# UW-ACL/SCPToolbox.jl

Measured on NVIDIA H100. Metric: SCP iterations/sec (batch), higher is better.
Workload: dtype f64

## Files before the change

scptoolbox.jl_b200/csrc/conic_ipm.cuh:

```cuda
#pragma once
#include <cuda_runtime.h>
#include <math_constants.h>

#include "conic_sn.cuh"

struct IpmProgram {
    int n, p, m, l, nsoc, nk, nnzL, nlevels, nwm, nnzA, nnzG;
    const int *soc_dim, *soc_off, *soc_woff;
    const int *A_rp, *A_ci, *G_rp, *G_ci;
    const int *At_rp, *At_ri, *At_vi, *Gt_rp, *Gt_ri, *Gt_vi;
    const int *iperm;
    const int *L_cp, *L_ri, *Lr_rp, *Lr_pos, *Lr_col;
    const int *lvl_ptr, *lvl_nodes;
    const int *as_ptr, *as_a, *as_b, *as_c, *as_src, *as_sign;
    const int4 *fw_item, *bw_item;
    const int4 *fwp_item, *bwp_item, *fa_item, *fb_item;
    SnProgram sn;
    HyProgram hy;
    int ysize;
    const int *sn_pos;
    const int *fa_lvl, *fa_R, *fb_lvl;
    const int *fwp_lvl, *bwp_lvl, *fwp_R, *bwp_R;
    const int2 *Lr_pc, *ft_op;
    const int4 *fwc_item, *bwc_item;
// ... 28 lines not shown
    double *xw, *yw, *zw, *sw;
    int *warm;
    double *rx, *ry, *rz, *lam, *wm, *socw, *soceta;
    double *dx, *dy, *dz, *ds, *dsa, *dza, *tm, *gm, *r1, *r2, *e1, *e2, *rhs, *Y, *Ls, *Lrow, *invD;
    double *part;
    double *pcnt;
    int vsmem;
    int psmem;
    double *pobj, *dobj, *res;
    int *status, *iters;
    const int *skip;
    int debug_kkt;
    int lvl_prof;
    int sn;
    long long *prof;
    double *trace;
    int trace_seed;
};

enum { IPM_OPTIMAL = 0, IPM_MAXIT = 1, IPM_NUMERICAL = 2, IPM_ALMOST = 3, IPM_PINF = 4, IPM_DINF = 5 };

#define IPM_MAXG 8
#define IPM_NT_MAX 1024

#ifdef CONIC_IPM_IMPL
struct Ctx {
    int G, sg, slot, nslots, tid, nwarps;
    int R, rr, isl, nisl;
    const int *s_lvl;
    int o_fal, o_faR, o_fbl;
    int o_fwl, o_bwl, o_fwR, o_bwR, o_vs;
    int Rmax;
    int *flag;
    long long t_fw, t_bw, t_ldl_n;
    long long *lprof;
    int sn;
    double *Ypanels;
    const struct SnArgs *s_sn;
    const struct HyArgs *s_hy;
    size_t ysize;
    const int *s_done;
    double *s_delta;
    int *s_bad;
    double rho_min, bad_abs;
    double *vs;
    double *Lrow;
    double *fpart, *spart;
    unsigned *pcnt;
    double reftol;
    const double *s_mu;
    double mu_tight;
    double *red;
    double *out;
};

template <int K>
__device__ __forceinline__ void seed_reduce(const Ctx &c, double (&v)[K], int op)
{
    const int lane = c.tid & 31, warp = c.tid >> 5;
    const int G = c.G;
#pragma unroll
    for (int k = 0; k < K; k++) {
        double a = v[k];
        for (int o = 16; o >= G; o >>= 1) {
            const double t = __shfl_xor_sync(0xffffffffu, a, o);
            a = (op == 0) ? a + t : ((op == 1) ? fmin(a, t) : fmax(a, t));
        }
        v[k] = a;
    }
    __syncthreads();
    if (lane < G) {
#pragma unroll
        for (int k = 0; k < K; k++) c.red[(k * (IPM_NT_MAX / 32) + warp) * IPM_MAXG + lane] = v[k];
    }
    __syncthreads();
    if (c.tid < G) {
#pragma unroll
        for (int k = 0; k < K; k++) {
            double a = c.red[(k * (IPM_NT_MAX / 32)) * IPM_MAXG + c.tid];
            for (int w = 1; w < c.nwarps; w++) {
                const double t = c.red[(k * (IPM_NT_MAX / 32) + w) * IPM_MAXG + c.tid];
                a = (op == 0) ? a + t : ((op == 1) ? fmin(a, t) : fmax(a, t));
            }
            c.out[k * IPM_MAXG + c.tid] = a;
        }
    }
    __syncthreads();
}

#define GI(e) ((size_t)(e) * G + sg)

__device__ __forceinline__ void set_lanes(Ctx &c, int R)
{
    const int sh = 31 - __clz(R);
    c.R = R; c.rr = c.slot & (R - 1); c.isl = c.slot >> sh; c.nisl = c.nslots >> sh;
}

__device__ __forceinline__ double lanes_sum(const Ctx &c, double a)
{
    for (int o = c.G; o < c.G * c.R; o <<= 1) a += __shfl_xor_sync(0xffffffffu, a, o);
    return a;
}

__device__ __forceinline__ double row_dot(const int *rp, const int *ci, const double *Mv, const double *x, int r,
                                          int G, int sg)
{
    double acc = 0.0;
    for (int k = rp[r]; k < rp[r + 1]; k++) acc = fma(Mv[GI(k)], x[GI(ci[k])], acc);
    return acc;
}
__device__ __forceinline__ double col_dot(const int *trp, const int *tri, const int *tvi, const double *Mv,
                                          const double *y, int v, int G, int sg)
{
    double acc = 0.0;
    for (int k = trp[v]; k < trp[v + 1]; k++) acc = fma(Mv[GI(tvi[k])], y[GI(tri[k])], acc);
    return acc;
}

__device__ void apply_winv2(const IpmProgram &P, const Ctx &c, const double *wm, const double *socw,
                            const double *soceta, const double *in, double *out)
{
    const int G = c.G, sg = c.sg;
    for (int r = c.slot; r < P.l; r += c.nslots) out[GI(r)] = wm[GI(r)] * in[GI(r)];
    for (int k = c.slot; k < P.nsoc; k += c.nslots) {
// ... 30 lines not shown
    for (int t = c.slot; t < ntgt; t += c.nslots) {
        double acc = dl * (double)P.as_sign[t];
        const int src = P.as_src[t];
        if (src >= 0) acc += Av[GI(src)];
        for (int k = P.as_ptr[t]; k < P.as_ptr[t + 1]; k++)
            acc = fma(Gv[GI(P.as_a[k])] * Gv[GI(P.as_b[k])], wmx[GI(P.as_c[k])], acc);
        if (D.sn) Y[(size_t)sg * c.ysize + P.sn_pos[t]] = acc;
        else Y[GI(t)] = acc;
    }
    __syncthreads();
}

#define IPM_FPF CONIC_FACTOR_PF
__device__ __forceinline__ bool ipm_split_done(double *part, unsigned *cnt, int4 e, double v, int G, int sg)
{
    part[e.w * G + sg] = v;
    __threadfence_block();
    const bool last = atomicAdd(&cnt[e.y * G + sg], 1u) == (unsigned)(e.z - e.y - 1);
    if (last) { __threadfence_block(); cnt[e.y * G + sg] = 0u; }
    return last;
}
__device__ __forceinline__ double ipm_split_sum(const double *part, int k0, int k1, double acc, int G, int sg)
{
    for (int k = k0; k < k1; k++) acc -= part[k * G + sg];
    return acc;
}
struct FactorArgs {
    const int4 *fa_item, *fb_item;
    const int2 *ft_op;
    const int4 *fb_cmb;
    double *Y, *Ls, *Lrow, *invD;
    double *part;
    int o_fal, o_faR, o_fbl;
    int nl, nnzLd, G, sg, slot, nslots;
    long long *lprof;
};
extern __shared__ int ipm_smem[];
__shared__ double ipm_s_delta[IPM_MAXG];
__shared__ int ipm_s_bad[IPM_MAXG];
__shared__ double ipm_s_reg[2];

__device__ __noinline__ void kkt_factor_levels(const FactorArgs a)
{
    __builtin_assume(__isGlobal(a.fa_item)); __builtin_assume(__isGlobal(a.fb_item)); __builtin_assume(__isGlobal(a.ft_op));
    __builtin_assume(__isGlobal(a.Y)); __builtin_assume(__isGlobal(a.Ls)); __builtin_assume(__isGlobal(a.Lrow));
    __builtin_assume(__isGlobal(a.invD));
    const int *fal = ipm_smem + a.o_fal, *faR = ipm_smem + a.o_faR, *fbl = ipm_smem + a.o_fbl;
    const int G = a.G, sg = a.sg, slot = a.slot, nslots = a.nslots;
    int t_tgt;
    int2 t_op[IPM_FPF];
    int i_tgt, i_k0, i_k1;
#define IPM_FA_ITEM(LV, OFF)                                                              \
    {                                                                                     \
        const int R_ = faR[LV], sh_ = 31 - __clz(R_);                                     \
        const int w_ = fal[LV] + (OFF) + (slot >> sh_);                                   \
        i_tgt = -1; i_k0 = 0; i_k1 = 0;                                                   \
        if ((OFF) < fal[(LV) + 1] - fal[LV] && w_ < fal[(LV) + 1]) {                      \
            const int4 it_ = a.fa_item[w_];                                               \
            i_tgt = it_.w ? ((it_.w - 1) | (1 << 30)) : it_.x;                              \
            i_k0 = it_.y + (slot & (R_ - 1)); i_k1 = it_.z;                               \
        }                                                                                 \
    }
#define IPM_FA_OPS(TGT, OP, R_)                                                           \
    {                                                                                     \
        TGT = i_tgt;                                                                      \
        _Pragma("unroll") for (int j = 0; j < IPM_FPF; j++) {                             \
            const int k_ = i_k0 + j * (R_);                                               \
            OP[j] = (i_tgt >= 0 && k_ < i_k1) ? a.ft_op[k_] : make_int2(-1, 0);           \
        }                                                                                 \
    }
    IPM_FA_ITEM(0, 0)
    IPM_FA_OPS(t_tgt, t_op, faR[0])
    IPM_FA_ITEM(0, (nslots >> (31 - __clz(faR[0]))))
    long long tl_ = a.lprof ? clock64() : 0;
    for (int lv = 0; lv < a.nl; lv++) {
        const int R = faR[lv], nisl = nslots >> (31 - __clz(R));
        const int nA = fal[lv + 1] - fal[lv];
        const int b0 = fbl[lv], b1 = fbl[lv + 1];
        int4 sc = make_int4(-1, 0, 0, 0), sr = make_int4(0, 0, 0, 0);
        if (b0 + slot < b1) { sc = a.fb_item[b0 + slot]; sr = a.fb_cmb[b0 + slot]; }
        for (int off = 0; off < nA; off += nisl) {
            double ya_[IPM_FPF], la_[IPM_FPF];
#pragma unroll
            for (int j = 0; j < IPM_FPF; j++) {
                const bool on_ = t_op[j].x >= 0;
                ya_[j] = on_ ? __ldcg(&a.Y[(size_t)t_op[j].x * G + sg]) : 0.0;
                la_[j] = on_ ? a.Lrow[(size_t)t_op[j].y * G + sg] : 0.0;
            }
            int n_tgt; int2 n_op[IPM_FPF];
            IPM_FA_OPS(n_tgt, n_op, R)
            IPM_FA_ITEM(lv, off + 2 * nisl)
            double part_ = 0.0;
#pragma unroll
            for (int j = 0; j < IPM_FPF; j++) part_ = fma(ya_[j], la_[j], part_);
            for (int o_ = G; o_ < G * R; o_ <<= 1) part_ += __shfl_xor_sync(0xffffffffu, part_, o_);
            if (t_tgt >= 0 && (slot & (R - 1)) == 0) {
                if (t_tgt >> 30) a.part[(t_tgt & 0x3fffffff) * G + sg] = part_;
                else { double *p_ = &a.Y[(size_t)t_tgt * G + sg]; *p_ = __ldcg(p_) - part_; }
            }
            t_tgt = n_tgt;
#pragma unroll
            for (int j = 0; j < IPM_FPF; j++) t_op[j] = n_op[j];
        }
        if (lv + 1 < a.nl) IPM_FA_ITEM(lv + 1, 0)
        __syncthreads();
        for (int w = b0 + slot; w < b1; w += nslots) {
            const double sgn = (sc.w & 1) ? 1.0 : -1.0;
            const bool isd = (sc.w & 2) != 0;
            double e = __ldcg(&a.Y[(size_t)sc.x * G + sg]);
            double d = isd ? 0.0 : __ldcg(&a.Y[(size_t)(a.nnzLd + sc.y) * G + sg]);
            const int4 cur = sc, cr = sr;
            if (w + nslots < b1) { sc = a.fb_item[w + nslots]; sr = a.fb_cmb[w + nslots]; }
            e = ipm_split_sum(a.part, cr.x, cr.y, e, G, sg);
            if (isd) d = e;
            else {
                d = ipm_split_sum(a.part, cr.z, cr.w, d, G, sg);
                if (cr.y > cr.x) a.Y[(size_t)cur.x * G + sg] = e;
                if (cur.w & 4) continue;
            }
            const double dl_ = ipm_s_delta[sg];
            if (!(sgn * d > 0.5 * dl_)) {
                if (isd && !(fabs(d) <= ipm_s_reg[1])) ipm_s_bad[sg] = 1;
                d = sgn * fmax(dl_, ipm_s_reg[0]);
            }
            const double inv = 1.0 / d;
            if (isd) a.invD[(size_t)cur.y * G + sg] = inv;
            else {
                const double lv_ = e * inv;
                a.Ls[(size_t)cur.x * G + sg] = lv_;
                a.Lrow[(size_t)cur.z * G + sg] = lv_;
            }
        }
        if (lv + 1 < a.nl) {
            const int Rn = faR[lv + 1];
            IPM_FA_OPS(t_tgt, t_op, Rn)
            IPM_FA_ITEM(lv + 1, (nslots >> (31 - __clz(Rn))))
        }
        __syncthreads();
        if (a.lprof) { const long long tn = clock64(); a.lprof[lv] += tn - tl_; tl_ = tn; }
    }
#undef IPM_FA_ITEM
#undef IPM_FA_OPS
}

struct SnArgs {
    SnProgram sn;
    double *Y, *invD, *vs;
    const int *s_done;
    const double *s_delta;
    int *s_bad;
    double rho_min, bad_abs;
    size_t ysize;
    int G, tid, nwarps, nls;
    long long *lprof;
};

template <int GS, class F>
__device__ __forceinline__ void sn_for_items(const SnArgs &a, int lv, int cls, F &&f)
{
    const int i0 = a.sn.cls_ptr[5 * lv + cls], nit = (a.sn.cls_ptr[5 * lv + cls + 1] - i0) * a.G;
    const int gsh = 31 - __clz(a.G);
    int unit, nunits;
    if (GS == 1) { unit = a.tid; nunits = a.nwarps * 32; }
    else { constexpr int GPW = 32 / (GS == 1 ? 32 : GS); unit = (a.tid >> 5) * GPW + ((a.tid & 31) / (GS == 1 ? 32 : GS)); nunits = a.nwarps * GPW; }
    int it = unit;
    int4 d0 = make_int4(0, 0, 0, 0), d1 = d0;
    if (it < nit) { const int q = 2 * (i0 + (it >> gsh)); d0 = a.sn.desc[q]; d1 = a.sn.desc[q + 1]; }
    while (it < nit) {
        const int sgi = it & (a.G - 1);
        const int4 c0 = d0, c1 = d1;
        const int nx = it + nunits;
        if (nx < nit) { const int q = 2 * (i0 + (nx >> gsh)); d0 = a.sn.desc[q]; d1 = a.sn.desc[q + 1]; }
        if (!a.s_done[sgi]) f(c0, c1, sgi);
        it = nx;
    }
// ... 25 lines not shown
}

template <int DIR>
__device__ __noinline__ void kkt_sweep_sn(const SnArgs *ap, int tid)
{
    SnArgs a = *ap;
    a.tid = tid;
    if (tid != 0) a.lprof = nullptr;
    const int G = a.G;
    double *vs = a.vs;
    long long tlp_ = a.lprof ? clock64() : 0;
    for (int st = 0; st < a.sn.nlevels; st++) {
        const int lv = DIR > 0 ? st : a.sn.nlevels - 1 - st;
        if (DIR > 0) {
            sn_for_items<1>(a, lv, 0, [&](const int4 d0, const int4 d1, int sgi) { sn1_forward_panel(a.sn, d0, d1, a.Y + (size_t)sgi * a.ysize, vs, G, sgi); });
            sn_for_items<8>(a, lv, 1, [&](const int4 d0, const int4 d1, int sgi) { sn_forward_panel<8>(a.sn, d0, d1, a.Y + (size_t)sgi * a.ysize, vs, G, sgi); });
            sn_for_items<16>(a, lv, 2, [&](const int4 d0, const int4 d1, int sgi) { sn_forward_panel<16>(a.sn, d0, d1, a.Y + (size_t)sgi * a.ysize, vs, G, sgi); });
            sn_for_items<32>(a, lv, 3, [&](const int4 d0, const int4 d1, int sgi) { sn_forward_panel<32>(a.sn, d0, d1, a.Y + (size_t)sgi * a.ysize, vs, G, sgi); });
        } else {
            sn_for_items<1>(a, lv, 0, [&](const int4 d0, const int4 d1, int sgi) { sn1_backward_panel(a.sn, d0, d1, a.Y + (size_t)sgi * a.ysize, vs, G, sgi); });
            sn_for_items<8>(a, lv, 1, [&](const int4 d0, const int4 d1, int sgi) { sn_backward_panel<8>(a.sn, d0, d1, a.Y + (size_t)sgi * a.ysize, vs, G, sgi); });
            sn_for_items<16>(a, lv, 2, [&](const int4 d0, const int4 d1, int sgi) { sn_backward_panel<16>(a.sn, d0, d1, a.Y + (size_t)sgi * a.ysize, vs, G, sgi); });
            sn_for_items<32>(a, lv, 3, [&](const int4 d0, const int4 d1, int sgi) { sn_backward_panel<32>(a.sn, d0, d1, a.Y + (size_t)sgi * a.ysize, vs, G, sgi); });
        }
        __syncthreads();
        if (a.lprof) { const long long tn = clock64(); a.lprof[(DIR > 0 ? 1 : 2) * a.nls + lv] += tn - tlp_; tlp_ = tn; }
    }
}

__device__ __forceinline__ void kkt_ldl_solve_sn(const IpmProgram &P, Ctx &c, const double *invD, double *v)
{
    const int G = c.G, sg = c.sg;
    double *vs = c.vs;
    const long long t0_ = clock64();
    for (int i = c.slot; i < P.nk; i += c.nslots) vs[i * G + sg] = v[GI(i)];
    __syncthreads();
    kkt_sweep_sn<1>(c.s_sn, c.tid);
    const long long t1_ = clock64();
    for (int i = c.slot; i < P.nk; i += c.nslots) vs[i * G + sg] *= invD[GI(i)];
    __syncthreads();
    kkt_sweep_sn<-1>(c.s_sn, c.tid);
    for (int i = c.slot; i < P.nk; i += c.nslots) v[GI(i)] = vs[i * G + sg];
    __syncthreads();
    const long long t2_ = clock64();
    c.t_fw += t1_ - t0_; c.t_bw += t2_ - t1_; c.t_ldl_n += 1;
}

struct HyArgs {
    HyProgram hy;
    double *Y, *Ls, *invD;
    const int *s_done;
    const double *s_delta;
    int *s_bad;
    double rho_min, bad_abs;
    int o_vs, nnzL, G, nwarps;
    long long *lprof;
};

template <class F>
__device__ __forceinline__ void hy_for_items(const HyArgs &a, int tl, int tid, F &&f)
{
    const int i0 = a.hy.tl_ptr[tl], nit = (a.hy.tl_ptr[tl + 1] - i0) * a.G;
    const int gsh = 31 - __clz(a.G);
    int it = tid >> 5;
    int4 d0 = make_int4(0, 0, 0, 0), d1 = d0;
    if (it < nit) { const int q = 2 * (i0 + (it >> gsh)); d0 = a.hy.desc[q]; d1 = a.hy.desc[q + 1]; }
    while (it < nit) {
        const int sgi = it & (a.G - 1);
        const int4 c0 = d0, c1 = d1;
        const int nx = it + a.nwarps;
        if (nx < nit) { const int q = 2 * (i0 + (nx >> gsh)); d0 = a.hy.desc[q]; d1 = a.hy.desc[q + 1]; }
        if (!a.s_done[sgi]) f(c0, c1, sgi);
        it = nx;
    }
}

__device__ __noinline__ void kkt_factor_top(const HyArgs *ap, int tid)
{
    const HyArgs a = *ap;
    long long *lp = (tid == 0) ? a.lprof : nullptr;
    long long tl_ = lp ? clock64() : 0;
    for (int tl = 0; tl < a.hy.ntl; tl++) {
        hy_for_items(a, tl, tid, [&](const int4 d0, const int4 d1, int sgi) {
            const double dl = a.s_delta[sgi];
            hy_factor_panel<32>(d0, d1, a.hy.upd_dst, a.Y, a.Ls, a.invD, a.nnzL, a.G, sgi, 0.5 * dl, fmax(dl, a.rho_min), a.bad_abs,
                                &a.s_bad[sgi]); });
        __syncthreads();
        if (lp) { const long long tn = clock64(); lp[tl] += tn - tl_; tl_ = tn; }
    }
}

template <int DIR>
__device__ __noinline__ void kkt_sweep_top(const HyArgs *ap, int tid)
{
    const HyArgs a = *ap;
    double *vs = (double *)(ipm_smem + a.o_vs);
    long long *lp = (tid == 0 && a.lprof) ? a.lprof + (DIR > 0 ? 1 : 2) * a.hy.ntl : nullptr;
    long long tl_ = lp ? clock64() : 0;
    for (int st = 0; st < a.hy.ntl; st++) {
        const int tl = DIR > 0 ? st : a.hy.ntl - 1 - st;
        if (DIR > 0) hy_for_items(a, tl, tid, [&](const int4 d0, const int4 d1, int sgi) { hy_forward_panel<32>(d0, d1, a.hy.rows, a.Ls, vs, a.G, sgi); });
        else hy_for_items(a, tl, tid, [&](const int4 d0, const int4 d1, int sgi) { hy_backward_panel<32>(d0, d1, a.hy.rows, a.Ls, vs, a.G, sgi); });
        __syncthreads();
        if (lp) { const long long tn = clock64(); lp[tl] += tn - tl_; tl_ = tn; }
    }
}

template <int SN>
__device__ __forceinline__ void kkt_factor(const IpmProgram &P, Ctx &c, double *Y, double *Ls, double *invD)
{
    if constexpr (SN == 1) { kkt_factor_sn(c.s_sn, c.tid); return; }
    FactorArgs a;
    a.fa_item = P.fa_item; a.fb_item = P.fb_item; a.ft_op = P.ft_op; a.fb_cmb = P.fb_cmb;
    a.Y = Y; a.Ls = Ls; a.Lrow = c.Lrow; a.invD = invD; a.part = c.fpart;
    a.o_fal = c.o_fal; a.o_faR = c.o_faR; a.o_fbl = c.o_fbl;
    a.nl = P.nlevels; a.nnzLd = P.nnzL; a.G = c.G; a.sg = c.sg; a.slot = c.slot; a.nslots = c.nslots;
    a.lprof = c.lprof;
    kkt_factor_levels(a);
    if constexpr (SN == 2) kkt_factor_top(c.s_hy, c.tid);
}

#define IPM_PF CONIC_SOLVE_PF
struct SweepArgs {
    const int4 *items;
    const int *idxarr;
    const double *vals;
    const int4 *cmb;
    double *part;
    unsigned *pcnt;
    int o_lvl, o_R, o_vs;
    int nl, lv0, G, sg, slot, nslots;
    long long *lprof;
};

template <int DIR>
__device__ __noinline__ void solve_sweep(const SweepArgs a)
{
    __builtin_assume(__isGlobal(a.items)); __builtin_assume(__isGlobal(a.idxarr)); __builtin_assume(__isGlobal(a.vals));
    const int *lvl = ipm_smem + a.o_lvl, *Rl = ipm_smem + a.o_R;
    double *vs = (double *)(ipm_smem + a.o_vs);
    const int G = a.G, sg = a.sg, slot = a.slot;
    const int nsteps = DIR > 0 ? a.nl - a.lv0 : a.lv0 + 1;
    if (nsteps <= 0) return;
    int i_node, i_k0, i_k1, i_R;
    int q_node;
    int q_idx[IPM_PF];
    double q_val[IPM_PF];
#define IPM_ITEM_LOAD(LV, OFF)                                                            \
    {                                                                                     \
        const int R_ = Rl[LV], sh_ = 31 - __clz(R_);                                      \
        const int w_ = lvl[LV] + (OFF) + (slot >> sh_);                                   \
        i_node = -1; i_R = R_; i_k0 = 0; i_k1 = 0;                                        \
        if (w_ < lvl[(LV) + 1]) {                                                         \
            const int4 it_ = a.items[w_];                                                 \
            i_node = it_.w ? ((it_.w - 1) | (1 << 30)) : it_.x;                             \
            i_k0 = it_.y + (slot & (R_ - 1)); i_k1 = it_.z;                               \
        }                                                                                 \
    }
#define IPM_VALS_LOAD()                                                                   \
    {                                                                                     \
        q_node = i_node;                                                                  \
        _Pragma("unroll") for (int j = 0; j < IPM_PF; j++) {                              \
            const int k_ = i_k0 + j * i_R;                                                \
            const bool on_ = i_node >= 0 && k_ < i_k1;                                    \
            q_idx[j] = on_ ? a.idxarr[k_] : 0;                                            \
            q_val[j] = on_ ? a.vals[(size_t)k_ * G + sg] : 0.0;                           \
        }                                                                                 \
    }
#define IPM_CONSUME(R)                                                                    \
    {                                                                                     \
        double part_ = 0.0;                                                               \
        _Pragma("unroll") for (int j = 0; j < IPM_PF; j++) part_ = fma(q_val[j], vs[q_idx[j] * G + sg], part_); \
        for (int o_ = G; o_ < G * (R); o_ <<= 1) part_ += __shfl_xor_sync(0xffffffffu, part_, o_); \
        if (q_node >= 0 && (slot & ((R) - 1)) == 0) {                                     \
            if (q_node >> 30) {                                                           \
                const int4 e_ = a.cmb[q_node & 0x3fffffff];                               \
                if (ipm_split_done(a.part, a.pcnt, e_, part_, G, sg))                     \
                    vs[e_.x * G + sg] = ipm_split_sum(a.part, e_.y, e_.z, vs[e_.x * G + sg], G, sg); \
            } else vs[q_node * G + sg] -= part_;                                          \
        }                                                                                 \
    }
    IPM_ITEM_LOAD(a.lv0, 0)
    IPM_VALS_LOAD()
    if (nsteps > 1) IPM_ITEM_LOAD(a.lv0 + DIR, 0) else i_node = -1;
    __syncthreads();
    long long tl_ = a.lprof ? clock64() : 0;
    for (int st = 0, lv = a.lv0; st < nsteps; st++, lv += DIR) {
        const int R = Rl[lv], nisl = a.nslots >> (31 - __clz(R));
        IPM_CONSUME(R)
        const int nit = lvl[lv + 1] - lvl[lv];
        if (nit > nisl) {
            const int sn = i_node, s0 = i_k0, s1 = i_k1, sR = i_R;
            for (int off = nisl; off < nit; off += nisl) {
                IPM_ITEM_LOAD(lv, off)
                IPM_VALS_LOAD()
                IPM_CONSUME(R)
            }
            i_node = sn; i_k0 = s0; i_k1 = s1; i_R = sR;
        }
        IPM_VALS_LOAD()
        if (st + 2 < nsteps) IPM_ITEM_LOAD(lv + 2 * DIR, 0) else i_node = -1;
        __syncthreads();
        if (a.lprof) { const long long tn = clock64(); a.lprof[lv] += tn - tl_; tl_ = tn; }
    }
#undef IPM_ITEM_LOAD
#undef IPM_VALS_LOAD
#undef IPM_CONSUME
}

template <int SN>
__device__ __forceinline__ void kkt_ldl_solve_smem(const IpmProgram &P, Ctx &c, const double *Ls, const double *invD, double *v)
{
    const int G = c.G, sg = c.sg;
    double *vs = c.vs;
    const long long t0_ = clock64();
    for (int i = c.slot; i < P.nk; i += c.nslots) vs[i * G + sg] = v[GI(i)];
    SweepArgs a;
    a.nl = P.nlevels; a.G = G; a.sg = sg; a.slot = c.slot; a.nslots = c.nslots; a.o_vs = c.o_vs; a.part = c.spart; a.pcnt = c.pcnt;
    a.items = P.fwp_item; a.idxarr = P.Lr_col; a.vals = c.Lrow; a.o_lvl = c.o_fwl; a.o_R = c.o_fwR; a.lv0 = 1;
    a.cmb = P.fwc_item;
    a.lprof = c.lprof ? c.lprof + P.nlevels : nullptr;
    solve_sweep<1>(a);
    if (P.nlevels <= 1) __syncthreads();
    if constexpr (SN == 2) kkt_sweep_top<1>(c.s_hy, c.tid);
    const long long t1_ = clock64();
    for (int i = c.slot; i < P.nk; i += c.nslots) vs[i * G + sg] *= invD[GI(i)];
    if constexpr (SN == 2) { __syncthreads(); kkt_sweep_top<-1>(c.s_hy, c.tid); }
    a.items = P.bwp_item; a.idxarr = P.L_ri; a.vals = Ls; a.o_lvl = c.o_bwl; a.o_R = c.o_bwR; a.lv0 = P.nlevels - 2;
    a.cmb = P.bwc_item;
    a.lprof = c.lprof ? c.lprof + 2 * P.nlevels : nullptr;
    solve_sweep<-1>(a);
    if (P.nlevels <= 1) __syncthreads();
    for (int i = c.slot; i < P.nk; i += c.nslots) v[GI(i)] = vs[i * G + sg];
    __syncthreads();
    const long long t2_ = clock64();
    c.t_fw += t1_ - t0_; c.t_bw += t2_ - t1_; c.t_ldl_n += 1;
}

template <int SN>
__device__ __forceinline__ void kkt_ldl_solve(const IpmProgram &P, Ctx &c, const double *Ls, const double *invD, double *v)
{
    if constexpr (SN == 1) { kkt_ldl_solve_sn(P, c, invD, v); return; }
    if (SN == 2 || c.vs) { kkt_ldl_solve_smem<SN>(P, c, Ls, invD, v); return; }
    set_lanes(c, c.Rmax);
    const int G = c.G, sg = c.sg;
    for (int lv = 0; lv < P.nlevels; lv++) {
        const int wend = c.s_lvl[lv + 1];
        for (int w0 = c.s_lvl[lv]; w0 < wend; w0 += c.nisl) {
            const int w = w0 + c.isl;
            const bool on = w < wend;
            int4 item = make_int4(0, 0, 0, 0);
            double part = 0.0, vi = 0.0;
            if (on) {
                item = P.fw_item[w];
                if (c.rr == 0) vi = v[GI(item.x)];
                const int k1 = item.z;
                int k = item.y + c.rr;
                for (; k + c.R < k1; k += 2 * c.R) {
                    const int2 a = P.Lr_pc[k], b = P.Lr_pc[k + c.R];
                    const double l0 = Ls[GI(a.x)], v0 = v[GI(a.y)], l1 = Ls[GI(b.x)], v1 = v[GI(b.y)];
                    part = fma(l0, v0, part);
                    part = fma(l1, v1, part);
                }
                if (k < k1) { const int2 a = P.Lr_pc[k]; part = fma(Ls[GI(a.x)], v[GI(a.y)], part); }
            }
            part = lanes_sum(c, part);
            if (on && c.rr == 0) v[GI(item.x)] = vi - part;
        }
        __syncthreads();
// ... 312 lines not shown
    __shared__ double s_red[10 * (IPM_NT_MAX / 32) * IPM_MAXG];
    __shared__ double s_out[10 * IPM_MAXG];
    __shared__ double s_nb[IPM_MAXG], s_nh[IPM_MAXG], s_nc[IPM_MAXG];
    __shared__ double s_mu[IPM_MAXG], s_sigmu[IPM_MAXG], s_alpha[IPM_MAXG], s_scale[IPM_MAXG];
    __shared__ int s_flag;
    __shared__ int s_done[IPM_MAXG], s_status[IPM_MAXG], s_iters[IPM_MAXG], s_alldone, s_save[IPM_MAXG], s_stall[IPM_MAXG];
    __shared__ double s_best[IPM_MAXG], s_bp[IPM_MAXG], s_bd[IPM_MAXG], s_br[3 * IPM_MAXG];
    __shared__ double s_alpha_d[IPM_MAXG];
    __shared__ int s_warm[IPM_MAXG], s_wsaved[IPM_MAXG], s_wsave[IPM_MAXG], s_allwarm, s_redo;
    __shared__ int s_skip[IPM_MAXG];
    double *const s_delta = ipm_s_delta;
    int *const s_bad = ipm_s_bad;
    __shared__ SnArgs s_snargs;
    __shared__ HyArgs s_hyargs;

    int *s_lv = ipm_smem;
    const int nl1 = P.nlevels + 1;
    for (int i = threadIdx.x; i <= P.nlevels; i += NT) {
        s_lv[i] = P.lvl_ptr[i]; s_lv[nl1 + i] = P.fa_lvl[i]; s_lv[2 * nl1 + i] = P.fb_lvl[i];
        s_lv[5 * nl1 + i] = P.fwp_lvl[i]; s_lv[6 * nl1 + i] = P.bwp_lvl[i];
    }
    for (int i = threadIdx.x; i < P.nlevels; i += NT) {
        s_lv[4 * nl1 + i] = P.fa_R[i]; s_lv[7 * nl1 + i] = P.fwp_R[i]; s_lv[8 * nl1 + i] = P.bwp_R[i];
    }
    Ctx c;
    c.s_lvl = s_lv;
    c.o_fal = nl1; c.o_fbl = 2 * nl1; c.o_faR = 4 * nl1;
    c.o_fwl = 5 * nl1; c.o_bwl = 6 * nl1; c.o_fwR = 7 * nl1; c.o_bwR = 8 * nl1;
    c.o_vs = (9 * (P.nlevels + 1) + 3) & ~3;
    c.vs = D.vsmem ? (double *)(s_lv + c.o_vs) : nullptr;
    c.G = D.G; c.tid = threadIdx.x; c.sg = c.tid % c.G; c.slot = c.tid / c.G; c.nslots = NT / c.G; c.nwarps = NT / 32;
    c.flag = &s_flag; c.reftol = O.reftol; c.s_mu = s_mu; c.mu_tight = O.mu_tight;
    c.Rmax = D.R;
    c.t_fw = c.t_bw = c.t_ldl_n = 0;
    c.lprof = (blockIdx.x == 0 && threadIdx.x == 0 && D.prof && D.lvl_prof) ? D.prof + 12 : nullptr;
    if (c.lprof) for (int i = 0; i < 3 * (P.nlevels + (SN == 2 ? P.hy.ntl : 0)); i++) c.lprof[i] = 0;
    set_lanes(c, c.Rmax);
    __syncthreads();
    c.red = s_red; c.out = s_out;
    const int G = c.G, sg = c.sg;
    const size_t g = (size_t)blockIdx.x + D.g0;
    const int seed = (int)g * G + sg;
    const bool live = seed < D.B;
    (void)live;

#define GP(arr, E) ((arr) + g * (size_t)(E) * G)
    double *Av = GP(D.Av, P.nnzA), *Gv = GP(D.Gv, P.nnzG), *cc = GP(D.c, P.n), *bb = GP(D.b, P.p), *hh = GP(D.h, P.m);
    double *eqD = GP(D.eqD, P.n), *eqA = GP(D.eqA, P.p), *eqG = GP(D.eqG, P.m);
    double *x = GP(D.x, P.n), *y = GP(D.y, P.p), *z = GP(D.z, P.m), *s = GP(D.s, P.m);
    double *xb = GP(D.xb, P.n), *yb = GP(D.yb, P.p), *zb = GP(D.zb, P.m), *sb = GP(D.sb, P.m);
    double *rx = GP(D.rx, P.n), *ry = GP(D.ry, P.p), *rz = GP(D.rz, P.m), *lam = GP(D.lam, P.m);
    double *wm = GP(D.wm, P.nwm), *socw = GP(D.socw, P.m - P.l + 1), *soceta = GP(D.soceta, P.nsoc + 1);
    double *dx = GP(D.dx, P.n), *dy = GP(D.dy, P.p), *dz = GP(D.dz, P.m), *ds = GP(D.ds, P.m);
    double *dsa = GP(D.dsa, P.m), *dza = GP(D.dza, P.m), *tm = GP(D.tm, P.m), *gm = GP(D.gm, P.m);
    double *r1 = GP(D.r1, P.n), *r2 = GP(D.r2, P.p);
    const int nm = (P.n > P.m ? P.n : P.m);
    double *e1 = GP(D.e1, nm), *e2 = GP(D.e2, P.p), *rhs = GP(D.rhs, P.nk);
    double *Y = GP(D.Y, P.ysize), *Ls = GP(D.Ls, P.nnzL + 1), *invD = GP(D.invD, P.nk);
    c.sn = D.sn; c.Ypanels = Y; c.ysize = (size_t)P.ysize;
    c.s_done = s_done; c.s_delta = s_delta; c.s_bad = s_bad; c.rho_min = O.rho_min; c.bad_abs = O.bad_abs;
    if (threadIdx.x == 0) { ipm_s_reg[0] = O.rho_min; ipm_s_reg[1] = O.bad_abs; }
    c.s_sn = &s_snargs;
    c.s_hy = &s_hyargs;
    if (SN == 2 && threadIdx.x == 0) {
        HyArgs a;
        a.hy = P.hy; a.Y = Y; a.Ls = Ls; a.invD = invD; a.s_done = s_done; a.s_delta = s_delta; a.s_bad = s_bad;
        a.rho_min = O.rho_min; a.bad_abs = O.bad_abs; a.o_vs = c.o_vs; a.nnzL = P.nnzL; a.G = D.G; a.nwarps = NT / 32;
        a.lprof = (blockIdx.x == 0 && D.prof && D.lvl_prof) ? D.prof + 12 + 3 * P.nlevels : nullptr;
        s_hyargs = a;
    }
    if (SN == 1 && threadIdx.x == 0) {
        SnArgs a;
        a.sn = P.sn; a.Y = Y; a.invD = invD; a.vs = c.vs; a.s_done = s_done; a.s_delta = s_delta; a.s_bad = s_bad;
        a.rho_min = O.rho_min; a.bad_abs = O.bad_abs; a.ysize = (size_t)P.ysize; a.G = D.G; a.tid = 0; a.nwarps = NT / 32;
        a.nls = P.nlevels; a.lprof = (blockIdx.x == 0 && D.prof && D.lvl_prof) ? D.prof + 12 : nullptr;
        s_snargs = a;
    }
    c.Lrow = GP(D.Lrow, P.nnzL + 1);
    if (D.psmem) {
        const int vw = 2 * (P.nk > P.npf ? P.nk : P.npf) * G;
        c.fpart = (double *)(s_lv + c.o_vs);
        c.spart = (double *)(s_lv + c.o_vs + vw);
        c.pcnt = (unsigned *)(s_lv + c.o_vs + vw + 2 * P.nps * G);
        for (int i = c.tid; i < P.nps * G; i += NT) c.pcnt[i] = 0u;
    } else {
        c.fpart = c.spart = GP(D.part, P.npart + 1);
        c.pcnt = (unsigned *)GP(D.pcnt, P.npart + 1);
    }
#undef GP

    long long pt[8] = {0, 0, 0, 0, 0, 0, 0, 0};
    long long n_fact = 0;
    long long n_retry = 0;
    long long tq = clock64();
    const long long tstart = tq;
#define PROF(i) { const long long tn = clock64(); pt[i] += tn - tq; tq = tn; }
    if (c.tid < G) {
        const int sd = (int)g * G + c.tid;
        const int sk = (sd >= D.B) || (D.skip && D.skip[sd]);
        s_skip[c.tid] = sk; s_done[c.tid] = sk;
        s_status[c.tid] = IPM_MAXIT; s_iters[c.tid] = 0; s_best[c.tid] = CUDART_INF; s_save[c.tid] = 0; s_stall[c.tid] = 0;
        s_delta[c.tid] = O.delta; s_bad[c.tid] = 0;
        s_mu[c.tid] = CUDART_INF;
        s_warm[c.tid] = (!sk && O.warm && D.warm && D.warm[sd]) ? 1 : 0;
        s_wsaved[c.tid] = 0; s_wsave[c.tid] = 0;
    }
    __syncthreads();
    {
        int all = 1;
        for (int q = 0; q < G; q++) all &= s_skip[q];
        if (all) return;
    }
    if (D.debug_kkt) {
        kkt_assemble(P, c, D, Av, Gv, wm, Y, 0.0);
        kkt_factor<SN>(P, c, Y, Ls, invD);
        kkt_ldl_solve<SN>(P, c, Ls, invD, rhs);
        if (c.tid < G && (int)g * G + c.tid < D.B) D.status[(int)g * G + c.tid] = s_bad[c.tid];
        return;
    }
#define IPM_FACTOR()                                                                               \
    for (int tr_ = 0;; tr_++) {                                                                    \
        if (c.tid < G) s_bad[c.tid] = 0;                                                           \
        kkt_assemble(P, c, D, Av, Gv, wm, Y, 0.0);                                                 \
        kkt_factor<SN>(P, c, Y, Ls, invD);                                                             \
        if (c.tid == 0) {                                                                          \
            int again_ = 0;                                                                        \
            for (int q = 0; q < G; q++)                                                            \
                if (s_bad[q] && !s_done[q] && s_delta[q] < O.delta_max) {                          \
                    s_delta[q] = fmin(s_delta[q] * O.delta_esc, O.delta_max); again_ = 1;          \
                }                                                                                  \
            s_flag = again_;                                                                       \
        }                                                                                          \
        __syncthreads();                                                                           \
        const int again_ = s_flag;                                                                 \
        __syncthreads();                                                                           \
        if (!again_ || tr_ >= 4) break;                                                            \
        n_retry++;                                                                                 \
    }
    if (O.equil > 0) equilibrate(P, c, Av, Gv, cc, bb, hh, eqD, eqA, eqG, O.equil);
    PROF(0)
    {
        double v[3] = {0.0, 0.0, 0.0};
        for (int i = c.slot; i < P.p; i += c.nslots) v[0] += bb[GI(i)] * bb[GI(i)];
        for (int i = c.slot; i < P.m; i += c.nslots) v[1] += hh[GI(i)] * hh[GI(i)];
        for (int i = c.slot; i < P.n; i += c.nslots) v[2] += cc[GI(i)] * cc[GI(i)];
        seed_reduce<3>(c, v, 0);
        if (c.tid < G) {
            s_nb[c.tid] = fmax(1.0, sqrt(s_out[0 * IPM_MAXG + c.tid]));
            s_nh[c.tid] = fmax(1.0, sqrt(s_out[1 * IPM_MAXG + c.tid]));
            s_nc[c.tid] = fmax(1.0, sqrt(s_out[2 * IPM_MAXG + c.tid]));
        }
        __syncthreads();
    }
    int tried_cold = 0;
restart_cold:
    if (c.tid == 0) {
        int all = 1;
        for (int q = 0; q < G; q++) all &= (s_warm[q] || s_skip[q]);
        s_allwarm = all;
    }
    __syncthreads();
    if (!s_allwarm) {
        set_identity_scaling(P, c, wm, socw, soceta);
        __syncthreads();
        IPM_FACTOR()
        for (int v = c.slot; v < P.n; v += c.nslots) r1[GI(v)] = 0.0;
        __syncthreads();
        kkt_solve<SN>(P, c, D, Av, Gv, wm, socw, soceta, r1, bb, hh, x, dy, dz, tm, gm, e1, e2, rhs, Ls, invD, O.nref);
        for (int r = c.slot; r < P.m; r += c.nslots) s[GI(r)] = -dz[GI(r)];
        __syncthreads();
// ... 119 lines not shown
            }
        }
        __syncthreads();
        if (s_save[sg]) {
            for (int i = c.slot; i < P.n; i += c.nslots) xb[GI(i)] = x[GI(i)];
            for (int i = c.slot; i < P.p; i += c.nslots) yb[GI(i)] = y[GI(i)];
            for (int i = c.slot; i < P.m; i += c.nslots) { zb[GI(i)] = z[GI(i)]; sb[GI(i)] = s[GI(i)]; }
        }
        if (s_wsave[sg]) {
            const bool eq = O.equil > 0;
            for (int i = c.slot; i < P.n; i += c.nslots) D.xw[g * (size_t)P.n * G + GI(i)] = eq ? x[GI(i)] * eqD[GI(i)] : x[GI(i)];
            for (int i = c.slot; i < P.p; i += c.nslots) D.yw[g * (size_t)P.p * G + GI(i)] = eq ? y[GI(i)] * eqA[GI(i)] : y[GI(i)];
            for (int i = c.slot; i < P.m; i += c.nslots) {
                const double e_ = eq ? eqG[GI(i)] : 1.0;
                D.zw[g * (size_t)P.m * G + GI(i)] = z[GI(i)] * e_;
                D.sw[g * (size_t)P.m * G + GI(i)] = s[GI(i)] / e_;
            }
        }
        __syncthreads();
        if (c.tid == 0) {
            int all = 1;
            for (int q = 0; q < G; q++) all &= (s_done[q] || ((int)g * G + q >= D.B));
            s_alldone = all;
        }
        __syncthreads();
        if (s_alldone) break;
        PROF(2)

        nt_scaling(P, c, s, z, lam, wm, socw, soceta);
        __syncthreads();
        PROF(3)
        IPM_FACTOR()
        PROF(4)
        n_fact++;

        for (int i = c.slot; i < P.n; i += c.nslots) r1[GI(i)] = -rx[GI(i)];
        for (int i = c.slot; i < P.p; i += c.nslots) r2[GI(i)] = -ry[GI(i)];
        for (int i = c.slot; i < P.m; i += c.nslots) ds[GI(i)] = -rz[GI(i)] + s[GI(i)];
        __syncthreads();
        PROF(6)
        kkt_solve<SN>(P, c, D, Av, Gv, wm, socw, soceta, r1, r2, ds, dx, dy, dza, tm, gm, e1, e2, rhs, Ls, invD, O.nref_aff);
        PROF(5)
        for (int i = c.slot; i < P.m; i += c.nslots) dsa[GI(i)] = -s[GI(i)] - gm[GI(i)];
        __syncthreads();
        {
            double a[2] = {cone_alpha_partial(P, c, s, dsa), cone_alpha_partial(P, c, z, dza)};
            seed_reduce<2>(c, a, 1);
            const double ap = fmin(1.0, s_out[sg]), ad = fmin(1.0, s_out[IPM_MAXG + sg]);
            double ma[1] = {0.0};
            for (int i = c.slot; i < P.m; i += c.nslots) ma[0] = fma(s[GI(i)] + ap * dsa[GI(i)], z[GI(i)] + ad * dza[GI(i)], ma[0]);
            seed_reduce<1>(c, ma, 0);
            if (c.tid < G) {
                double r = s_out[c.tid] / (deg * s_mu[c.tid]);
                r = fmin(1.0, fmax(0.0, r));
                if (!(r == r)) r = 1.0;
                const double sig = r * r * r;
                s_sigmu[c.tid] = sig * s_mu[c.tid];
                s_scale[c.tid] = 1.0 - sig;
            }
            __syncthreads();
        }
        combined_tmp(P, c, s, z, lam, socw, soceta, dsa, dza, s_sigmu, tm);
        __syncthreads();
        {
            const double sc = s_scale[sg];
            for (int i = c.slot; i < P.n; i += c.nslots) r1[GI(i)] = -sc * rx[GI(i)];
            for (int i = c.slot; i < P.p; i += c.nslots) r2[GI(i)] = -sc * ry[GI(i)];
// ... 17 lines not shown
                s_alpha_d[c.tid] = s_done[c.tid] ? 0.0 : fmin(1.0, 0.99 * s_out[IPM_MAXG + c.tid]);
            }
            __syncthreads();
        }
        for (int bt = 0; bt < 12; bt++) {
            double mg[2] = {cone_margin_partial(P, c, s, ds, s_alpha[sg]), cone_margin_partial(P, c, z, dz, s_alpha_d[sg])};
            seed_reduce<2>(c, mg, 1);
            if (c.tid == 0) s_alldone = 1;
            __syncthreads();
            if (c.tid < G) {
                if (s_alpha[c.tid] > 0.0 && !(s_out[c.tid] > 0.0)) { s_alpha[c.tid] *= 0.5; s_alldone = 0; }
                if (s_alpha_d[c.tid] > 0.0 && !(s_out[IPM_MAXG + c.tid] > 0.0)) { s_alpha_d[c.tid] *= 0.5; s_alldone = 0; }
            }
            __syncthreads();
            const int okall = s_alldone;
            __syncthreads();
            if (okall) break;
        }
        {
            const double ap = s_alpha[sg], ad = s_alpha_d[sg];
            if (ap > 0.0) {
                for (int i = c.slot; i < P.n; i += c.nslots) x[GI(i)] += ap * dx[GI(i)];
                for (int i = c.slot; i < P.m; i += c.nslots) s[GI(i)] += ap * ds[GI(i)];
            }
            if (ad > 0.0) {
                for (int i = c.slot; i < P.p; i += c.nslots) y[GI(i)] += ad * dy[GI(i)];
                for (int i = c.slot; i < P.m; i += c.nslots) z[GI(i)] += ad * dz[GI(i)];
            }
        }
        __syncthreads();
        PROF(6)
    }
    if (blockIdx.x == 0 && threadIdx.x == 0 && D.prof) {
        pt[7] = clock64() - tstart;
        for (int i = 0; i < 8; i++) D.prof[i] = pt[i];
        D.prof[8] = c.t_fw; D.prof[9] = c.t_bw; D.prof[10] = c.t_ldl_n; D.prof[11] = n_fact | (n_retry << 32);
    }
#undef PROF
    __syncthreads();
    if (c.tid == 0) {
        int redo = 0;
        if (!tried_cold)
            for (int q = 0; q < G; q++)
                if (s_warm[q] && !s_skip[q] && s_status[q] != IPM_OPTIMAL && s_status[q] != IPM_PINF && s_status[q] != IPM_DINF &&
                    !(s_best[q] <= 10.0 * fmax(O.feastol, O.reltol)))
                    redo = 1;
        s_redo = redo;
    }
    __syncthreads();
    if (s_redo) {
        tried_cold = 1;
        if (c.tid < G) {
            const int q = c.tid;
            s_done[q] = s_skip[q]; s_status[q] = IPM_MAXIT; s_iters[q] = 0; s_best[q] = CUDART_INF; s_save[q] = 0; s_stall[q] = 0;
            s_delta[q] = O.delta; s_bad[q] = 0; s_warm[q] = 0; s_wsaved[q] = 0; s_wsave[q] = 0;
        }
        __syncthreads();
        goto restart_cold;
    }
    __syncthreads();
    if (c.tid < G && s_status[c.tid] != IPM_OPTIMAL && s_status[c.tid] != IPM_PINF && s_status[c.tid] != IPM_DINF) {
        if (s_best[c.tid] <= 10.0 * fmax(O.feastol, O.reltol)) s_status[c.tid] = IPM_OPTIMAL;
        else if (s_best[c.tid] <= 5e-5) s_status[c.tid] = IPM_ALMOST;
    }
    __syncthreads();
    if (s_best[sg] < CUDART_INF) {
        for (int i = c.slot; i < P.n; i += c.nslots) x[GI(i)] = xb[GI(i)];
        for (int i = c.slot; i < P.p; i += c.nslots) y[GI(i)] = yb[GI(i)];
        for (int i = c.slot; i < P.m; i += c.nslots) { z[GI(i)] = zb[GI(i)]; s[GI(i)] = sb[GI(i)]; }
// ... 20 lines not shown
```

Before: 688.3.

## Move kernel args and profiling state to shared memory, template factor on G

Moves the per-thread profiling counters and clock stamps into shared memory updated only by thread 0. FactorArgs and SweepArgs are built once into shared memory instead of being passed by value, and HyArgs are taken by reference. The level factorization is templated on G so index math uses compile-time shifts and 32-bit offsets. The aim is lower register pressure and less argument copying in noinline device functions, at the cost of shared-memory reads for the arguments and possible int overflow in the now unwidened index products.

```diff
diff --git a/scptoolbox.jl_b200/csrc/conic_ipm.cuh b/scptoolbox.jl_b200/csrc/conic_ipm.cuh
--- a/scptoolbox.jl_b200/csrc/conic_ipm.cuh
+++ b/scptoolbox.jl_b200/csrc/conic_ipm.cuh
@@ -84,7 +84,6 @@
     int o_fwl, o_bwl, o_fwR, o_bwR, o_vs;
     int Rmax;
     int *flag;
-    long long t_fw, t_bw, t_ldl_n;
     long long *lprof;
     int sn;
     double *Ypanels;
@@ -142,6 +141,9 @@
 
 #define GI(e) ((size_t)(e) * G + sg)
 
+__shared__ long long ipm_s_prof[16];
+#define IPM_STAMP(k) { if (threadIdx.x == 0) ipm_s_prof[k] = clock64(); }
+
 __device__ __forceinline__ void set_lanes(Ctx &c, int R)
 {
     const int sh = 31 - __clz(R);
@@ -238,21 +240,25 @@
     double *Y, *Ls, *Lrow, *invD;
     double *part;
     int o_fal, o_faR, o_fbl;
-    int nl, nnzLd, G, sg, slot, nslots;
+    int nl, nnzLd, G, nslots;
     long long *lprof;
 };
 extern __shared__ int ipm_smem[];
 __shared__ double ipm_s_delta[IPM_MAXG];
 __shared__ int ipm_s_bad[IPM_MAXG];
 __shared__ double ipm_s_reg[2];
-
-__device__ __noinline__ void kkt_factor_levels(const FactorArgs a)
-{
+__shared__ FactorArgs ipm_fa;
+__shared__ long long ipm_lvl_t;
+
+template <int G>
+__device__ __forceinline__ void kkt_factor_levels_g()
+{
+    const FactorArgs &a = ipm_fa;
     __builtin_assume(__isGlobal(a.fa_item)); __builtin_assume(__isGlobal(a.fb_item)); __builtin_assume(__isGlobal(a.ft_op));
     __builtin_assume(__isGlobal(a.Y)); __builtin_assume(__isGlobal(a.Ls)); __builtin_assume(__isGlobal(a.Lrow));
     __builtin_assume(__isGlobal(a.invD));
+    const int sg = threadIdx.x & (G - 1), slot = threadIdx.x / G, nslots = a.nslots;
     const int *fal = ipm_smem + a.o_fal, *faR = ipm_smem + a.o_faR, *fbl = ipm_smem + a.o_fbl;
-    const int G = a.G, sg = a.sg, slot = a.slot, nslots = a.nslots;
     int t_tgt;
     int2 t_op[IPM_FPF];
     int i_tgt, i_k0, i_k1;
@@ -278,20 +284,17 @@
     IPM_FA_ITEM(0, 0)
     IPM_FA_OPS(t_tgt, t_op, faR[0])
     IPM_FA_ITEM(0, (nslots >> (31 - __clz(faR[0]))))
-    long long tl_ = a.lprof ? clock64() : 0;
+    if (threadIdx.x == 0 && a.lprof) ipm_lvl_t = clock64();
     for (int lv = 0; lv < a.nl; lv++) {
         const int R = faR[lv], nisl = nslots >> (31 - __clz(R));
         const int nA = fal[lv + 1] - fal[lv];
-        const int b0 = fbl[lv], b1 = fbl[lv + 1];
-        int4 sc = make_int4(-1, 0, 0, 0), sr = make_int4(0, 0, 0, 0);
-        if (b0 + slot < b1) { sc = a.fb_item[b0 + slot]; sr = a.fb_cmb[b0 + slot]; }
         for (int off = 0; off < nA; off += nisl) {
             double ya_[IPM_FPF], la_[IPM_FPF];
 #pragma unroll
             for (int j = 0; j < IPM_FPF; j++) {
                 const bool on_ = t_op[j].x >= 0;
-                ya_[j] = on_ ? __ldcg(&a.Y[(size_t)t_op[j].x * G + sg]) : 0.0;
-                la_[j] = on_ ? a.Lrow[(size_t)t_op[j].y * G + sg] : 0.0;
+                ya_[j] = on_ ? __ldcg(&a.Y[t_op[j].x * G + sg]) : 0.0;
+                la_[j] = on_ ? a.Lrow[t_op[j].y * G + sg] : 0.0;
             }
             int n_tgt; int2 n_op[IPM_FPF];
             IPM_FA_OPS(n_tgt, n_op, R)
@@ -302,26 +305,29 @@
             for (int o_ = G; o_ < G * R; o_ <<= 1) part_ += __shfl_xor_sync(0xffffffffu, part_, o_);
             if (t_tgt >= 0 && (slot & (R - 1)) == 0) {
                 if (t_tgt >> 30) a.part[(t_tgt & 0x3fffffff) * G + sg] = part_;
-                else { double *p_ = &a.Y[(size_t)t_tgt * G + sg]; *p_ = __ldcg(p_) - part_; }
+                else { double *p_ = &a.Y[t_tgt * G + sg]; *p_ = __ldcg(p_) - part_; }
             }
             t_tgt = n_tgt;
 #pragma unroll
             for (int j = 0; j < IPM_FPF; j++) t_op[j] = n_op[j];
         }
+        const int b0 = fbl[lv], b1 = fbl[lv + 1];
+        int4 sc = make_int4(-1, 0, 0, 0), sr = make_int4(0, 0, 0, 0);
+        if (b0 + slot < b1) { sc = a.fb_item[b0 + slot]; sr = a.fb_cmb[b0 + slot]; }
         if (lv + 1 < a.nl) IPM_FA_ITEM(lv + 1, 0)
         __syncthreads();
         for (int w = b0 + slot; w < b1; w += nslots) {
             const double sgn = (sc.w & 1) ? 1.0 : -1.0;
             const bool isd = (sc.w & 2) != 0;
-            double e = __ldcg(&a.Y[(size_t)sc.x * G + sg]);
-            double d = isd ? 0.0 : __ldcg(&a.Y[(size_t)(a.nnzLd + sc.y) * G + sg]);
+            double e = __ldcg(&a.Y[sc.x * G + sg]);
+            double d = isd ? 0.0 : __ldcg(&a.Y[(a.nnzLd + sc.y) * G + sg]);
             const int4 cur = sc, cr = sr;
             if (w + nslots < b1) { sc = a.fb_item[w + nslots]; sr = a.fb_cmb[w + nslots]; }
             e = ipm_split_sum(a.part, cr.x, cr.y, e, G, sg);
             if (isd) d = e;
             else {
                 d = ipm_split_sum(a.part, cr.z, cr.w, d, G, sg);
-                if (cr.y > cr.x) a.Y[(size_t)cur.x * G + sg] = e;
+                if (cr.y > cr.x) a.Y[cur.x * G + sg] = e;
                 if (cur.w & 4) continue;
             }
             const double dl_ = ipm_s_delta[sg];
@@ -330,11 +336,11 @@
                 d = sgn * fmax(dl_, ipm_s_reg[0]);
             }
             const double inv = 1.0 / d;
-            if (isd) a.invD[(size_t)cur.y * G + sg] = inv;
+            if (isd) a.invD[cur.y * G + sg] = inv;
             else {
                 const double lv_ = e * inv;
-                a.Ls[(size_t)cur.x * G + sg] = lv_;
-                a.Lrow[(size_t)cur.z * G + sg] = lv_;
+                a.Ls[cur.x * G + sg] = lv_;
+                a.Lrow[cur.z * G + sg] = lv_;
             }
         }
         if (lv + 1 < a.nl) {
@@ -343,10 +349,19 @@
             IPM_FA_ITEM(lv + 1, (nslots >> (31 - __clz(Rn))))
         }
         __syncthreads();
-        if (a.lprof) { const long long tn = clock64(); a.lprof[lv] += tn - tl_; tl_ = tn; }
+        if (threadIdx.x == 0 && a.lprof) { const long long tn = clock64(); a.lprof[lv] += tn - ipm_lvl_t; ipm_lvl_t = tn; }
     }
 #undef IPM_FA_ITEM
 #undef IPM_FA_OPS
+}
+__device__ __noinline__ void kkt_factor_levels()
+{
+    switch (ipm_fa.G) {
+        case 1: kkt_factor_levels_g<1>(); break;
+        case 2: kkt_factor_levels_g<2>(); break;
+        case 4: kkt_factor_levels_g<4>(); break;
+        default: kkt_factor_levels_g<8>(); break;
+    }
 }
 
 struct SnArgs {
@@ -438,18 +453,17 @@
 {
     const int G = c.G, sg = c.sg;
     double *vs = c.vs;
-    const long long t0_ = clock64();
+    IPM_STAMP(15)
     for (int i = c.slot; i < P.nk; i += c.nslots) vs[i * G + sg] = v[GI(i)];
     __syncthreads();
     kkt_sweep_sn<1>(c.s_sn, c.tid);
-    const long long t1_ = clock64();
+    if (c.tid == 0) { const long long t1_ = clock64(); ipm_s_prof[8] += t1_ - ipm_s_prof[15]; ipm_s_prof[15] = t1_; }
     for (int i = c.slot; i < P.nk; i += c.nslots) vs[i * G + sg] *= invD[GI(i)];
     __syncthreads();
     kkt_sweep_sn<-1>(c.s_sn, c.tid);
     for (int i = c.slot; i < P.nk; i += c.nslots) v[GI(i)] = vs[i * G + sg];
     __syncthreads();
-    const long long t2_ = clock64();
-    c.t_fw += t1_ - t0_; c.t_bw += t2_ - t1_; c.t_ldl_n += 1;
+    if (c.tid == 0) { ipm_s_prof[9] += clock64() - ipm_s_prof[15]; ipm_s_prof[10] += 1; }
 }
 
 struct HyArgs {
@@ -483,7 +497,7 @@
 
 __device__ __noinline__ void kkt_factor_top(const HyArgs *ap, int tid)
 {
-    const HyArgs a = *ap;
+    const HyArgs &a = *ap;
     long long *lp = (tid == 0) ? a.lprof : nullptr;
     long long tl_ = lp ? clock64() : 0;
     for (int tl = 0; tl < a.hy.ntl; tl++) {
@@ -499,7 +513,7 @@
 template <int DIR>
 __device__ __noinline__ void kkt_sweep_top(const HyArgs *ap, int tid)
 {
-    const HyArgs a = *ap;
+    const HyArgs &a = *ap;
     double *vs = (double *)(ipm_smem + a.o_vs);
     long long *lp = (tid == 0 && a.lprof) ? a.lprof + (DIR > 0 ? 1 : 2) * a.hy.ntl : nullptr;
     long long tl_ = lp ? clock64() : 0;
@@ -513,16 +527,10 @@
 }
 
 template <int SN>
-__device__ __forceinline__ void kkt_factor(const IpmProgram &P, Ctx &c, double *Y, double *Ls, double *invD)
+__device__ __forceinline__ void kkt_factor(const Ctx &c)
 {
     if constexpr (SN == 1) { kkt_factor_sn(c.s_sn, c.tid); return; }
-    FactorArgs a;
-    a.fa_item = P.fa_item; a.fb_item = P.fb_item; a.ft_op = P.ft_op; a.fb_cmb = P.fb_cmb;
-    a.Y = Y; a.Ls = Ls; a.Lrow = c.Lrow; a.invD = invD; a.part = c.fpart;
-    a.o_fal = c.o_fal; a.o_faR = c.o_faR; a.o_fbl = c.o_fbl;
-    a.nl = P.nlevels; a.nnzLd = P.nnzL; a.G = c.G; a.sg = c.sg; a.slot = c.slot; a.nslots = c.nslots;
-    a.lprof = c.lprof;
-    kkt_factor_levels(a);
+    kkt_factor_levels();
     if constexpr (SN == 2) kkt_factor_top(c.s_hy, c.tid);
 }
 
@@ -535,17 +543,19 @@
     double *part;
     unsigned *pcnt;
     int o_lvl, o_R, o_vs;
-    int nl, lv0, G, sg, slot, nslots;
+    int nl, lv0, G, nslots;
     long long *lprof;
 };
+__shared__ SweepArgs ipm_sw[2];
 
 template <int DIR>
-__device__ __noinline__ void solve_sweep(const SweepArgs a)
-{
+__device__ __noinline__ void solve_sweep()
+{
+    const SweepArgs &a = ipm_sw[DIR > 0 ? 0 : 1];
     __builtin_assume(__isGlobal(a.items)); __builtin_assume(__isGlobal(a.idxarr)); __builtin_assume(__isGlobal(a.vals));
     const int *lvl = ipm_smem + a.o_lvl, *Rl = ipm_smem + a.o_R;
     double *vs = (double *)(ipm_smem + a.o_vs);
-    const int G = a.G, sg = a.sg, slot = a.slot;
+    const int G = a.G, sg = threadIdx.x & (G - 1), slot = threadIdx.x >> (31 - __clz(G));
     const int nsteps = DIR > 0 ? a.nl - a.lv0 : a.lv0 + 1;
     if (nsteps <= 0) return;
     int i_node, i_k0, i_k1, i_R;
@@ -590,7 +600,7 @@
     IPM_VALS_LOAD()
     if (nsteps > 1) IPM_ITEM_LOAD(a.lv0 + DIR, 0) else i_node = -1;
     __syncthreads();
-    long long tl_ = a.lprof ? clock64() : 0;
+    if (threadIdx.x == 0 && a.lprof) ipm_lvl_t = clock64();
     for (int st = 0, lv = a.lv0; st < nsteps; st++, lv += DIR) {
         const int R = Rl[lv], nisl = a.nslots >> (31 - __clz(R));
         IPM_CONSUME(R)
@@ -607,7 +617,7 @@
         IPM_VALS_LOAD()
         if (st + 2 < nsteps) IPM_ITEM_LOAD(lv + 2 * DIR, 0) else i_node = -1;
         __syncthreads();
-        if (a.lprof) { const long long tn = clock64(); a.lprof[lv] += tn - tl_; tl_ = tn; }
+        if (threadIdx.x == 0 && a.lprof) { const long long tn = clock64(); a.lprof[lv] += tn - ipm_lvl_t; ipm_lvl_t = tn; }
     }
 #undef IPM_ITEM_LOAD
 #undef IPM_VALS_LOAD
@@ -619,28 +629,19 @@
 {
     const int G = c.G, sg = c.sg;
     double *vs = c.vs;
-    const long long t0_ = clock64();
+    IPM_STAMP(15)
     for (int i = c.slot; i < P.nk; i += c.nslots) vs[i * G + sg] = v[GI(i)];
-    SweepArgs a;
-    a.nl = P.nlevels; a.G = G; a.sg = sg; a.slot = c.slot; a.nslots = c.nslots; a.o_vs = c.o_vs; a.part = c.spart; a.pcnt = c.pcnt;
-    a.items = P.fwp_item; a.idxarr = P.Lr_col; a.vals = c.Lrow; a.o_lvl = c.o_fwl; a.o_R = c.o_fwR; a.lv0 = 1;
-    a.cmb = P.fwc_item;
-    a.lprof = c.lprof ? c.lprof + P.nlevels : nullptr;
-    solve_sweep<1>(a);
+    solve_sweep<1>();
     if (P.nlevels <= 1) __syncthreads();
     if constexpr (SN == 2) kkt_sweep_top<1>(c.s_hy, c.tid);
-    const long long t1_ = clock64();
+    if (c.tid == 0) { const long long t1_ = clock64(); ipm_s_prof[8] += t1_ - ipm_s_prof[15]; ipm_s_prof[15] = t1_; }
     for (int i = c.slot; i < P.nk; i += c.nslots) vs[i * G + sg] *= invD[GI(i)];
     if constexpr (SN == 2) { __syncthreads(); kkt_sweep_top<-1>(c.s_hy, c.tid); }
-    a.items = P.bwp_item; a.idxarr = P.L_ri; a.vals = Ls; a.o_lvl = c.o_bwl; a.o_R = c.o_bwR; a.lv0 = P.nlevels - 2;
-    a.cmb = P.bwc_item;
-    a.lprof = c.lprof ? c.lprof + 2 * P.nlevels : nullptr;
-    solve_sweep<-1>(a);
+    solve_sweep<-1>();
     if (P.nlevels <= 1) __syncthreads();
     for (int i = c.slot; i < P.nk; i += c.nslots) v[GI(i)] = vs[i * G + sg];
     __syncthreads();
-    const long long t2_ = clock64();
-    c.t_fw += t1_ - t0_; c.t_bw += t2_ - t1_; c.t_ldl_n += 1;
+    if (c.tid == 0) { ipm_s_prof[9] += clock64() - ipm_s_prof[15]; ipm_s_prof[10] += 1; }
 }
 
 template <int SN>
@@ -1019,7 +1020,6 @@
     c.G = D.G; c.tid = threadIdx.x; c.sg = c.tid % c.G; c.slot = c.tid / c.G; c.nslots = NT / c.G; c.nwarps = NT / 32;
     c.flag = &s_flag; c.reftol = O.reftol; c.s_mu = s_mu; c.mu_tight = O.mu_tight;
     c.Rmax = D.R;
-    c.t_fw = c.t_bw = c.t_ldl_n = 0;
     c.lprof = (blockIdx.x == 0 && threadIdx.x == 0 && D.prof && D.lvl_prof) ? D.prof + 12 : nullptr;
     if (c.lprof) for (int i = 0; i < 3 * (P.nlevels + (SN == 2 ? P.hy.ntl : 0)); i++) c.lprof[i] = 0;
     set_lanes(c, c.Rmax);
@@ -1074,14 +1074,32 @@
         c.fpart = c.spart = GP(D.part, P.npart + 1);
         c.pcnt = (unsigned *)GP(D.pcnt, P.npart + 1);
     }
+    if (SN != 1 && threadIdx.x == 0) {
+        FactorArgs a;
+        a.fa_item = P.fa_item; a.fb_item = P.fb_item; a.ft_op = P.ft_op; a.fb_cmb = P.fb_cmb;
+        a.Y = Y; a.Ls = Ls; a.Lrow = c.Lrow; a.invD = invD; a.part = c.fpart;
+        a.o_fal = c.o_fal; a.o_faR = c.o_faR; a.o_fbl = c.o_fbl;
+        a.nl = P.nlevels; a.nnzLd = P.nnzL; a.G = G; a.nslots = c.nslots;
+        a.lprof = c.lprof;
+        ipm_fa = a;
+        SweepArgs w;
+        w.nl = P.nlevels; w.G = G; w.nslots = c.nslots; w.o_vs = c.o_vs; w.part = c.spart; w.pcnt = c.pcnt;
+        w.items = P.fwp_item; w.idxarr = P.Lr_col; w.vals = c.Lrow; w.o_lvl = c.o_fwl; w.o_R = c.o_fwR; w.lv0 = 1;
+        w.cmb = P.fwc_item;
+        w.lprof = c.lprof ? c.lprof + P.nlevels : nullptr;
+        ipm_sw[0] = w;
+        w.items = P.bwp_item; w.idxarr = P.L_ri; w.vals = Ls; w.o_lvl = c.o_bwl; w.o_R = c.o_bwR; w.lv0 = P.nlevels - 2;
+        w.cmb = P.bwc_item;
+        w.lprof = c.lprof ? c.lprof + 2 * P.nlevels : nullptr;
+        ipm_sw[1] = w;
+    }
 #undef GP
 
-    long long pt[8] = {0, 0, 0, 0, 0, 0, 0, 0};
-    long long n_fact = 0;
-    long long n_retry = 0;
-    long long tq = clock64();
-    const long long tstart = tq;
-#define PROF(i) { const long long tn = clock64(); pt[i] += tn - tq; tq = tn; }
+    if (threadIdx.x == 0) {
+        for (int i = 0; i < 13; i++) ipm_s_prof[i] = 0;
+        ipm_s_prof[13] = ipm_s_prof[14] = clock64();
+    }
+#define PROF(i) { if (threadIdx.x == 0) { const long long tn = clock64(); ipm_s_prof[i] += tn - ipm_s_prof[13]; ipm_s_prof[13] = tn; } }
     if (c.tid < G) {
         const int sd = (int)g * G + c.tid;
         const int sk = (sd >= D.B) || (D.skip && D.skip[sd]);
@@ -1100,7 +1118,7 @@
     }
     if (D.debug_kkt) {
         kkt_assemble(P, c, D, Av, Gv, wm, Y, 0.0);
-        kkt_factor<SN>(P, c, Y, Ls, invD);
+        kkt_factor<SN>(c);
         kkt_ldl_solve<SN>(P, c, Ls, invD, rhs);
         if (c.tid < G && (int)g * G + c.tid < D.B) D.status[(int)g * G + c.tid] = s_bad[c.tid];
         return;
@@ -1109,7 +1127,7 @@
     for (int tr_ = 0;; tr_++) {                                                                    \
         if (c.tid < G) s_bad[c.tid] = 0;                                                           \
         kkt_assemble(P, c, D, Av, Gv, wm, Y, 0.0);                                                 \
-        kkt_factor<SN>(P, c, Y, Ls, invD);                                                             \
+        kkt_factor<SN>(c);                                                                         \
         if (c.tid == 0) {                                                                          \
             int again_ = 0;                                                                        \
             for (int q = 0; q < G; q++)                                                            \
@@ -1122,7 +1140,7 @@
         const int again_ = s_flag;                                                                 \
         __syncthreads();                                                                           \
         if (!again_ || tr_ >= 4) break;                                                            \
-        n_retry++;                                                                                 \
+        if (c.tid == 0) ipm_s_prof[12]++;                                                          \
     }
     if (O.equil > 0) equilibrate(P, c, Av, Gv, cc, bb, hh, eqD, eqA, eqG, O.equil);
     PROF(0)
@@ -1308,7 +1326,7 @@
         PROF(3)
         IPM_FACTOR()
         PROF(4)
-        n_fact++;
+        if (c.tid == 0) ipm_s_prof[11]++;
 
         for (int i = c.slot; i < P.n; i += c.nslots) r1[GI(i)] = -rx[GI(i)];
         for (int i = c.slot; i < P.p; i += c.nslots) r2[GI(i)] = -ry[GI(i)];
@@ -1392,9 +1410,9 @@
         PROF(6)
     }
     if (blockIdx.x == 0 && threadIdx.x == 0 && D.prof) {
-        pt[7] = clock64() - tstart;
-        for (int i = 0; i < 8; i++) D.prof[i] = pt[i];
-        D.prof[8] = c.t_fw; D.prof[9] = c.t_bw; D.prof[10] = c.t_ldl_n; D.prof[11] = n_fact | (n_retry << 32);
+        ipm_s_prof[7] = clock64() - ipm_s_prof[14];
+        for (int i = 0; i < 11; i++) D.prof[i] = ipm_s_prof[i];
+        D.prof[11] = ipm_s_prof[11] | (ipm_s_prof[12] << 32);
     }
 #undef PROF
     __syncthreads();
```

Result: faster. 765.1 (median of 6 runs) (+11.2%).
